# nage/indy-plenum

Hardware: AMD Instinct MI355X
Metric: Ed25519 verifies/sec at 1/2/4/8 MI355X vs libsodium on host cores (higher is better)
Workload: dtype u32; 1 GPU; C2: 1M Ed25519 request signatures per GPU, distinct keys, 256 B payloads, ~5% tampered (BASELINE.json configs[1]); signatures_per_gpu=1000000, msg_bytes=256, key_pool=distinct, key_cache=off, parallelism=single GPU

## Files before the change

indy-plenum_amd/csrc/pv_lattice.h:

```cpp
#pragma once
#include <stdint.h>
#include <math.h>
#include "pv_scalar.h"

namespace pv {

constexpr int HS_WORDS = 5;
constexpr int HS_T = 6;
constexpr uint32_t HS_NONE = 0, HS_HALF = 1, HS_DEFER = 2;

PV_HD uint32_t sc_8L(int i) {
  const uint32_t v[8] = {0xe7ae9f68u, 0xc09318d2u, 0x17bce6b2u, 0xa6f7cef5u, 0u, 0u, 0u, 0x80000000u};
  return v[i];
}

PV_HD double words_to_f64(const uint32_t r[8]) {
  double x = (double)r[7];
#pragma unroll
  for (int k = 6; k >= 0; --k) x = x * 4294967296.0 + (double)r[k];
  return x;
}

PV_HD bool ge2_128(const uint32_t r[8]) { return (r[4] | r[5] | r[6] | r[7]) != 0; }

PV_HD bool ge8(const uint32_t a[8], const uint32_t b[8]) {
  bool gt = false, decided = false;
#pragma unroll
  for (int k = 7; k >= 0; --k) {
    if (!decided && a[k] != b[k]) {
      gt = a[k] > b[k];
      decided = true;
    }
  }
  return !decided || gt;
}

PV_HD void add8(uint32_t a[8], const uint32_t b[8]) {
#if defined(__HIP_DEVICE_COMPILE__)
  unsigned c = 0;
#pragma unroll
  for (int k = 0; k < 8; ++k) a[k] = __builtin_addc(a[k], b[k], c, &c);
#else
  uint64_t c = 0;
#pragma unroll
  for (int k = 0; k < 8; ++k) {
    c += (uint64_t)a[k] + b[k];
    a[k] = (uint32_t)c;
    c >>= 32;
  }
#endif
}

PV_HD void sub8(uint32_t a[8], const uint32_t b[8]) {
#if defined(__HIP_DEVICE_COMPILE__)
  unsigned bw = 0;
#pragma unroll
  for (int k = 0; k < 8; ++k) a[k] = __builtin_subc(a[k], b[k], bw, &bw);
#else
  uint32_t br = 0;
#pragma unroll
  for (int k = 0; k < 8; ++k) {
    const uint64_t d = (uint64_t)a[k] - b[k] - br;
    a[k] = (uint32_t)d;
    br = (uint32_t)(d >> 63);
  }
#endif
}

PV_HD bool submul8(uint32_t a[8], const uint32_t b[8], uint32_t q) {
#if defined(__HIP_DEVICE_COMPILE__)
  uint32_t lo[8], hi[8];
#pragma unroll
  for (int k = 0; k < 8; ++k) {
    const uint64_t p = (uint64_t)q * b[k];
    lo[k] = (uint32_t)p;
    hi[k] = (uint32_t)(p >> 32);
  }
  unsigned b1 = 0, b2 = 0;
#pragma unroll
  for (int k = 0; k < 8; ++k) {
    unsigned o1, o2;
    const uint32_t t = __builtin_subc(a[k], lo[k], b1, &o1);
    a[k] = __builtin_subc(t, k ? hi[k - 1] : 0u, b2, &o2);
    b1 = o1;
    b2 = o2;
  }
  return (hi[7] | b1 | b2) != 0;
#else
  uint64_t pc = 0;
  uint32_t br = 0;
#pragma unroll
  for (int k = 0; k < 8; ++k) {
    const uint64_t p = (uint64_t)q * b[k] + pc;
    pc = p >> 32;
    const uint64_t d = (uint64_t)a[k] - (uint32_t)p - br;
    a[k] = (uint32_t)d;
    br = (uint32_t)(d >> 63);
  }
  return (pc + br) != 0;
#endif
}

PV_HD void addmul_t(uint32_t t[HS_T], const uint32_t u[HS_T], uint32_t q) {
#if defined(__HIP_DEVICE_COMPILE__)
  uint32_t lo[HS_T], hi[HS_T];
#pragma unroll
  for (int k = 0; k < HS_T; ++k) {
    const uint64_t p = (uint64_t)q * u[k];
    lo[k] = (uint32_t)p;
    hi[k] = (uint32_t)(p >> 32);
  }
  unsigned c1 = 0, c2 = 0;
#pragma unroll
  for (int k = 0; k < HS_T; ++k) {
    const uint32_t x = __builtin_addc(t[k], lo[k], c1, &c1);
    t[k] = __builtin_addc(x, k ? hi[k - 1] : 0u, c2, &c2);
  }
#else
  uint64_t c = 0;
#pragma unroll
  for (int k = 0; k < HS_T; ++k) {
    const uint64_t p = (uint64_t)q * u[k] + t[k] + c;
    t[k] = (uint32_t)p;
    c = p >> 32;
  }
#endif
}

PV_HD void add_t(uint32_t t[HS_T], const uint32_t u[HS_T]) {
#if defined(__HIP_DEVICE_COMPILE__)
  unsigned cc = 0;
#pragma unroll
  for (int k = 0; k < HS_T; ++k) t[k] = __builtin_addc(t[k], u[k], cc, &cc);
#else
  uint64_t c = 0;
#pragma unroll
  for (int k = 0; k < HS_T; ++k) {
    c += (uint64_t)t[k] + u[k];
    t[k] = (uint32_t)c;
    c >>= 32;
  }
#endif
}

PV_HD void sub_t(uint32_t t[HS_T], const uint32_t u[HS_T]) {
#if defined(__HIP_DEVICE_COMPILE__)
  unsigned bw = 0;
#pragma unroll
  for (int k = 0; k < HS_T; ++k) t[k] = __builtin_subc(t[k], u[k], bw, &bw);
#else
  uint32_t br = 0;
#pragma unroll
  for (int k = 0; k < HS_T; ++k) {
    const uint64_t d = (uint64_t)t[k] - u[k] - br;
    t[k] = (uint32_t)d;
    br = (uint32_t)(d >> 63);
  }
#endif
}

PV_HD double quot_est(double a, double b) {
#if defined(__HIP_DEVICE_COMPILE__)
  double r = __builtin_amdgcn_rcp(b);
  r = fma(r, fma(-b, r, 1.0), r);
  r = fma(r, fma(-b, r, 1.0), r);
  return floor(a * r);
#else
  return floor(a / b);
#endif
}

PV_HD bool euclid_step(uint32_t ra[8], uint32_t ta[HS_T], const uint32_t rb[8], const uint32_t tb[HS_T]) {
  const double qd = quot_est(words_to_f64(ra), words_to_f64(rb));
  if (!(qd < 4294967294.0)) return false;
  const uint32_t q = (uint32_t)qd;
  if (submul8(ra, rb, q)) {
    add8(ra, rb);
    addmul_t(ta, tb, q);
    sub_t(ta, tb);
  } else {
    addmul_t(ta, tb, q);
    if (ge8(ra, rb)) {
      sub8(ra, rb);
      add_t(ta, tb);
    }
  }
  return true;
}

PV_HD bool fits132(const uint32_t* v, int nw) {
  uint32_t hi = 0;
  for (int k = HS_WORDS; k < nw; ++k) hi |= v[k];
  if (hi) return false;
  uint64_t c = 0;
#pragma unroll
  for (int k = 0; k < 4; ++k) c = ((uint64_t)v[k] + 0x88888888u + c) >> 32;
  return (uint64_t)v[4] + 8u + c < 16u;
}

PV_HD uint32_t half_scalars(uint32_t c[HS_WORDS], uint32_t d[HS_WORDS], bool& c_neg, const uint32_t h[8]) {
  uint32_t ra[8], rb[8], ta[HS_T], tb[HS_T];
#pragma unroll
  for (int k = 0; k < 8; ++k) {
    ra[k] = sc_8L(k);
    rb[k] = h[k];
  }
#pragma unroll
  for (int k = 0; k < HS_T; ++k) ta[k] = tb[k] = 0;
  tb[0] = 1;
  uint32_t odd = 1;
  int trips = 0;
#pragma unroll 1
  for (;;) {
    if (!ge2_128(rb)) break;
    if (++trips > 96 || !euclid_step(ra, ta, rb, tb)) return HS_DEFER;
    odd ^= 1u;
    if (!ge2_128(ra)) {
#pragma unroll
      for (int k = 0; k < 8; ++k) {
        const uint32_t x = ra[k];
        ra[k] = rb[k];
        rb[k] = x;
      }
#pragma unroll
      for (int k = 0; k < HS_T; ++k) {
        const uint32_t x = ta[k];
        ta[k] = tb[k];
        tb[k] = x;
      }
      break;
    }
    if (!euclid_step(rb, tb, ra, ta)) return HS_DEFER;
    odd ^= 1u;
  }
  if (tb[0] & 1u) {
    c_neg = odd == 0;
#pragma unroll
    for (int k = 0; k < HS_WORDS; ++k) {
      c[k] = rb[k];
      d[k] = tb[k];
    }
    return HS_HALF;
  }
  if (!fits132(ra, 8)) {
    if ((rb[0] | rb[1] | rb[2] | rb[3]) == 0) return HS_DEFER;
    const double kd = ceil((words_to_f64(ra) - 2.5e39) / words_to_f64(rb));
    if (!(kd < 4294967294.0)) return HS_DEFER;
    const uint32_t k = kd > 0.0 ? (uint32_t)kd : 0u;
    if (submul8(ra, rb, k)) return HS_DEFER;
    addmul_t(ta, tb, k);
    if (!fits132(ra, 8)) {
      sub8(ra, rb);
      add_t(ta, tb);
    }
    if (!fits132(ra, 8)) return HS_DEFER;
  }
  if (!fits132(ta, HS_T)) return HS_DEFER;
  c_neg = odd == 1;
#pragma unroll
  for (int k = 0; k < HS_WORDS; ++k) {
    c[k] = ra[k];
    d[k] = ta[k];
  }
  return HS_HALF;
}

PV_HD void hs_offset(uint32_t v[HS_WORDS]) {
  uint64_t c = 0;
#pragma unroll
  for (int k = 0; k < HS_WORDS; ++k) {
    c += (uint64_t)v[k] + (k < 4 ? 0x88888888u : 0x8u);
    v[k] = (uint32_t)c;
    c >>= 32;
  }
}

PV_HD void sc_mul_small(uint32_t out[8], const uint32_t d[HS_WORDS], const uint32_t S[8]) {
  uint32_t x[16];
  uint64_t carry = 0;
#pragma unroll
  for (int k = 0; k < 16; ++k) {
    uint64_t acc = carry & 0xffffffffu;
    uint64_t acchi = carry >> 32;
#pragma unroll
    for (int i = 0; i < HS_WORDS; ++i) {
      const int j = k - i;
      if (j >= 0 && j < 8) {
        const uint64_t p = mul32x32(d[i], S[j]);
        acc += p & 0xffffffffu;
        acchi += p >> 32;
      }
    }
    acchi += acc >> 32;
    x[k] = (uint32_t)acc;
    carry = acchi;
  }
  sc_reduce64(out, x);
}

}
```

Measured before the change: 108.3 million verifies/s.

## Replace full-precision Euclid in half-scalar reduction with Lehmer-style batched steps

```diff
diff --git a/indy-plenum_amd/csrc/pv_lattice.h b/indy-plenum_amd/csrc/pv_lattice.h
--- a/indy-plenum_amd/csrc/pv_lattice.h
+++ b/indy-plenum_amd/csrc/pv_lattice.h
@@ -198,7 +198,200 @@
   return (uint64_t)v[4] + 8u + c < 16u;
 }
 
-PV_HD uint32_t half_scalars(uint32_t c[HS_WORDS], uint32_t d[HS_WORDS], bool& c_neg, const uint32_t h[8]) {
+
+PV_HD void mul8_lo(uint32_t out[8], const uint32_t b[8], uint32_t q) {
+#if defined(__HIP_DEVICE_COMPILE__)
+  uint32_t lo[8], hi[8];
+#pragma unroll
+  for (int k = 0; k < 8; ++k) {
+    const uint64_t p = (uint64_t)q * b[k];
+    lo[k] = (uint32_t)p;
+    hi[k] = (uint32_t)(p >> 32);
+  }
+  unsigned c = 0;
+  out[0] = lo[0];
+#pragma unroll
+  for (int k = 1; k < 8; ++k) out[k] = __builtin_addc(lo[k], hi[k - 1], c, &c);
+#else
+  uint64_t c = 0;
+#pragma unroll
+  for (int k = 0; k < 8; ++k) {
+    c += (uint64_t)q * b[k];
+    out[k] = (uint32_t)c;
+    c >>= 32;
+  }
+#endif
+}
+
+PV_HD void mul_t(uint32_t out[HS_T], const uint32_t u[HS_T], uint32_t q) {
+#if defined(__HIP_DEVICE_COMPILE__)
+  uint32_t lo[HS_T], hi[HS_T];
+#pragma unroll
+  for (int k = 0; k < HS_T; ++k) {
+    const uint64_t p = (uint64_t)q * u[k];
+    lo[k] = (uint32_t)p;
+    hi[k] = (uint32_t)(p >> 32);
+  }
+  unsigned c = 0;
+  out[0] = lo[0];
+#pragma unroll
+  for (int k = 1; k < HS_T; ++k) out[k] = __builtin_addc(lo[k], hi[k - 1], c, &c);
+#else
+  uint64_t c = 0;
+#pragma unroll
+  for (int k = 0; k < HS_T; ++k) {
+    c += (uint64_t)q * u[k];
+    out[k] = (uint32_t)c;
+    c >>= 32;
+  }
+#endif
+}
+
+PV_HD double quot_low(double x, double y) {
+  const double k = 1.0 - 0x1p-40;
+#if defined(__HIP_DEVICE_COMPILE__)
+  double r = __builtin_amdgcn_rcp(y);
+  r = fma(r, fma(-y, r, 1.0), r);
+  r = fma(r, fma(-y, r, 1.0), r);
+  return floor(x * r * k);
+#else
+  return floor(x / y * k);
+#endif
+}
+
+PV_HD void lead64(uint64_t& x0, uint64_t& x1, uint64_t& lim, const uint32_t ra[8], const uint32_t rb[8]) {
+  uint32_t a2 = ra[4], a1 = ra[3], a0 = ra[2], b2 = rb[4], b1 = rb[3], b0 = rb[2], w = 4;
+#pragma unroll
+  for (int k = 5; k < 8; ++k) {
+    const bool nz = ra[k] != 0;
+    a2 = nz ? ra[k] : a2;
+    a1 = nz ? ra[k - 1] : a1;
+    a0 = nz ? ra[k - 2] : a0;
+    b2 = nz ? rb[k] : b2;
+    b1 = nz ? rb[k - 1] : b1;
+    b0 = nz ? rb[k - 2] : b0;
+    w = nz ? (uint32_t)k : w;
+  }
+  const uint32_t lz = (uint32_t)__builtin_clz(a2 | 1u);
+  x0 = ((((uint64_t)a2 << 32) | a1) << lz) | ((uint64_t)a0 >> (32u - lz));
+  x1 = ((((uint64_t)b2 << 32) | b1) << lz) | ((uint64_t)b0 >> (32u - lz));
+  lim = w >= 6 ? 1u : (uint64_t)1 << (lz + (w == 4 ? 32u : 0u));
+}
+
+PV_HD bool lehmer_step(uint64_t& x0, double& f0, uint32_t& u0, uint32_t& v0, uint64_t x1, double f1, uint32_t u1,
+                       uint32_t v1, uint64_t need) {
+  bool go = x1 - v1 >= need;
+  const double qd = quot_low(f0, f1);
+  go &= qd < 4294967280.0;
+  uint32_t q = (uint32_t)(go ? qd : 0.0);
+  uint64_t x2 = x0 - q * x1;
+  const bool up = x2 >= x1;
+  x2 -= up ? x1 : 0u;
+  q += up ? 1u : 0u;
+  const uint64_t u2 = u0 + (uint64_t)q * u1, v2 = v0 + (uint64_t)q * v1;
+  go &= (v2 >> 32) == 0;
+  go &= x2 >= v2;
+  go &= x1 - x2 >= v1 + v2;
+  if (go) {
+    x0 = x2;
+    f0 = (double)x2;
+    u0 = (uint32_t)u2;
+    v0 = (uint32_t)v2;
+  }
+  return go;
+}
+
+struct LehmerNoProbe {
+  PV_HD void round() {}
+  PV_HD void full_step() {}
+};
+
+template <class Probe>
+PV_HD bool reduce_pair(uint32_t ra[8], uint32_t rb[8], uint32_t ta[HS_T], uint32_t tb[HS_T], uint32_t& odd,
+                       Probe& probe) {
+  int steps = 0;
+#pragma unroll 1
+  while (ge2_128(rb)) {
+    if (steps > 192) return false;
+    probe.round();
+    uint64_t x0, x1, lim;
+    lead64(x0, x1, lim, ra, rb);
+    uint32_t u0 = 1, v0 = 0, u1 = 0, v1 = 1;
+    uint32_t k = 0;
+    uint64_t need = 0;
+    double f0 = (double)x0, f1 = (double)x1;
+#pragma unroll 1
+    for (;;) {
+      if (!lehmer_step(x0, f0, u0, v0, x1, f1, u1, v1, need)) break;
+      need = lim;
+      ++k;
+      if (!lehmer_step(x1, f1, u1, v1, x0, f0, u0, v0, need)) break;
+      ++k;
+    }
+    if (k & 1u) {
+      const uint64_t x = x0;
+      x0 = x1;
+      x1 = x;
+      const uint32_t u = u0, v = v0;
+      u0 = u1;
+      u1 = u;
+      v0 = v1;
+      v1 = v;
+    }
+    if (k == 0) {
+      probe.full_step();
+      if (!euclid_step(ra, ta, rb, tb)) return false;
+#pragma unroll
+      for (int j = 0; j < 8; ++j) {
+        const uint32_t x = ra[j];
+        ra[j] = rb[j];
+        rb[j] = x;
+      }
+#pragma unroll
+      for (int j = 0; j < HS_T; ++j) {
+        const uint32_t x = ta[j];
+        ta[j] = tb[j];
+        tb[j] = x;
+      }
+      odd ^= 1u;
+      steps += 1;
+      continue;
+    }
+    const bool ev = (k & 1u) == 0;
+    uint32_t pa[8], pb[8], na[8], nb[8];
+#pragma unroll
+    for (int j = 0; j < 8; ++j) {
+      pa[j] = ev ? ra[j] : rb[j];
+      pb[j] = ev ? rb[j] : ra[j];
+    }
+    mul8_lo(na, pa, ev ? u0 : v0);
+    (void)submul8(na, pb, ev ? v0 : u0);
+    mul8_lo(nb, pb, ev ? v1 : u1);
+    (void)submul8(nb, pa, ev ? u1 : v1);
+    uint32_t ma[HS_T], mb[HS_T];
+    mul_t(ma, ta, u0);
+    addmul_t(ma, tb, v0);
+    mul_t(mb, ta, u1);
+    addmul_t(mb, tb, v1);
+#pragma unroll
+    for (int j = 0; j < 8; ++j) {
+      ra[j] = na[j];
+      rb[j] = nb[j];
+    }
+#pragma unroll
+    for (int j = 0; j < HS_T; ++j) {
+      ta[j] = ma[j];
+      tb[j] = mb[j];
+    }
+    odd ^= k & 1u;
+    steps += (int)k;
+  }
+  return true;
+}
+
+template <class Probe>
+PV_HD uint32_t half_scalars_probe(uint32_t c[HS_WORDS], uint32_t d[HS_WORDS], bool& c_neg, const uint32_t h[8],
+                                  Probe& probe) {
   uint32_t ra[8], rb[8], ta[HS_T], tb[HS_T];
 #pragma unroll
   for (int k = 0; k < 8; ++k) {
@@ -209,30 +402,7 @@
   for (int k = 0; k < HS_T; ++k) ta[k] = tb[k] = 0;
   tb[0] = 1;
   uint32_t odd = 1;
-  int trips = 0;
-#pragma unroll 1
-  for (;;) {
-    if (!ge2_128(rb)) break;
-    if (++trips > 96 || !euclid_step(ra, ta, rb, tb)) return HS_DEFER;
-    odd ^= 1u;
-    if (!ge2_128(ra)) {
-#pragma unroll
-      for (int k = 0; k < 8; ++k) {
-        const uint32_t x = ra[k];
-        ra[k] = rb[k];
-        rb[k] = x;
-      }
-#pragma unroll
-      for (int k = 0; k < HS_T; ++k) {
-        const uint32_t x = ta[k];
-        ta[k] = tb[k];
-        tb[k] = x;
-      }
-      break;
-    }
-    if (!euclid_step(rb, tb, ra, ta)) return HS_DEFER;
-    odd ^= 1u;
-  }
+  if (!reduce_pair(ra, rb, ta, tb, odd, probe)) return HS_DEFER;
   if (tb[0] & 1u) {
     c_neg = odd == 0;
 #pragma unroll
@@ -265,6 +435,11 @@
   return HS_HALF;
 }
 
+PV_HD uint32_t half_scalars(uint32_t c[HS_WORDS], uint32_t d[HS_WORDS], bool& c_neg, const uint32_t h[8]) {
+  LehmerNoProbe probe;
+  return half_scalars_probe(c, d, c_neg, h, probe);
+}
+
 PV_HD void hs_offset(uint32_t v[HS_WORDS]) {
   uint64_t c = 0;
 #pragma unroll
```

New measurement: 108.2 million verifies/s, median of 2. About the same (-0.1%).
